# focegueda1998/CALM-ViT-DTE

Hardware: AMD Instinct MI355X
Metric: training images/sec (224^2, bs=256/GPU) (higher is better)
Workload: dtype f32; 1 GPU; CALM-ViT small224 cls, 224x224x3 synthetic, bs=256/GPU, fp32 matmuls, fwd+loss+bwd+clip+AdamW; batch resident in HBM when the timed region starts (the trainer's H2D copy of the batch is excluded); global_batch=256, parallelism=dp1, world=1, backend=none (single process), hipgraph=False

## Files before the change

calm-vit-dte_amd/_lib.py:

```python
import ctypes as C
import os

HERE = os.path.dirname(os.path.abspath(__file__))
LIB_PATH = os.environ.get("CALM_VIT_LIB") or os.path.join(HERE, "libcalmvit_hip.so")

ACT_NONE, ACT_GELU, ACT_GELU_BWD = 0, 1, 2
F32 = 0
ST_F32, ST_BF16, ST_FP8_E4M3, ST_FP8_E5M2 = 0, 1, 2, 3
E_INVAL, E_LAYOUT, E_UNSUPP = -1, -2, -3
ABI_VERSION = 7

_p = C.c_void_p
_i32 = C.c_int32
_i64 = C.c_int64
_f32 = C.c_float


class GemmArgs(C.Structure):
    _fields_ = [
        ("A", _p), ("B", _p), ("C", _p),
        ("M", _i32), ("N", _i32), ("K", _i32),
        ("batch0", _i32), ("batch1", _i32),
        ("a_rs", _i64), ("a_cs", _i64), ("a_b0", _i64), ("a_b1", _i64),
        ("b_rs", _i64), ("b_cs", _i64), ("b_b0", _i64), ("b_b1", _i64),
# ... 49 lines not shown
    "calm_gemm": (_i32, [C.POINTER(GemmArgs), _p]),
    "calm_gemm_workspace_bytes": (_i64, [C.POINTER(GemmArgs)]),
    "calm_gemm_set_option": (C.c_int, [_i32, _i32]),
    "calm_gemm_describe": (_i32, [C.POINTER(GemmArgs), C.POINTER(GemmPlan)]),
    "calm_reduce_scratch_floats": (_i64, [_i32, _i64, _i32]),
    "calm_layernorm_fwd": (_i32, [_p, _p, _p, _p, _p, _i64, _i32, _f32, _i32, _p]),
    "calm_layernorm_bwd": (_i32, [_p, _p, _p, _p, _p, _p, _p, _p, _i64, _i32, _i32, _p, _p]),
    "calm_cast_chunk_elems": (_i32, []),
    "calm_cast_bf16": (_i32, [_p, _p, _i32, _p]),
    "calm_cast_bf16_one": (_i32, [_p, _p, _i64, _p]),
    "calm_cast_f32_one": (_i32, [_p, _p, _i64, _p]),
    "calm_quantize_fp8": (_i32, [_p, _i32, _i64, _p, _i32, _p, _p]),
    "calm_transpose_u8": (_i32, [_p, _p, _i32, _i32, _p]),
    "calm_rope_fwd": (_i32, [_p, _p, _p, _p, _p, _i32, _i32, _i32, _i32, _i32, _i32, _i32, _i32, _p]),
    "calm_rope_bwd": (_i32, [_p, _p, _p, _p, _p, _p, _i32, _i32, _i32, _i32, _i32, _i32, _i32, _i32, _i32, _p, _p]),
    "calm_softmax_fwd": (_i32, [_p, _i64, _i32, _p]),
    "calm_softmax_bwd": (_i32, [_p, _p, _i64, _i32, _p]),
    "calm_softmax_bwd_heads": (_i32, [_p, _p, _p, _i32, _i32, _i32, _i32, _p]),
    "calm_sum_heads": (_i32, [_p, _p, _i32, _i32, _i64, _p]),
    "calm_attention_fwd_supported": (_i32, [_i32, _i32, _i32, _i32]),
    "calm_attention_fwd": (_i32, [_p] * 15 + [_i32] * 5 + [_p]),
    "calm_attention_bwd_preferred": (_i32, [_i32, _i32, _i32, _i32]),
    "calm_attention_bwd": (_i32, [_p] * 10 + [_i32] * 5 + [_p]),
    "calm_attention_fwd_lse": (_i32, [_p] * 15 + [_i32] * 5 + [_p]),
    "calm_attention_bwd_lse_scratch_bytes": (_i64, [_i32] * 5),
    "calm_attention_bwd_lse": (_i32, [_p] * 7 + [_i64] + [_p] * 4 + [_i32] * 5 + [_p]),
    "calm_attention16_supported": (_i32, [_i32, _i32, _i32]),
    "calm_attention16_fwd": (_i32, [_p] * 16 + [_i32] * 4 + [_p]),
    "calm_attention16_bwd": (_i32, [_p] * 13 + [_i32] * 4 + [_p]),
    "calm_latent_fwd": (_i32, [_p, _p, _p, _p, _p, _i64, _i32, _p, _p]),
    "calm_latent_bwd": (_i32, [_p, _p, _p, _p, _p, _p, _i64, _i32, _p]),
    "calm_sn_plan": (_i32, [C.POINTER(SnLayer), _i32, _p, C.POINTER(SnPlanInfo)]),
    "calm_sn_power_iter": (_i32, [_p, C.POINTER(SnPlanInfo), _i32, _f32, _p, _p]),
    "calm_sn_weight_bwd": (_i32, [_p, _p, _p, _p, _p, _p, _p, _p, _i32, _i32, _p, _p]),
    "calm_optim_chunk_elems": (_i32, []),
    "calm_optim_step": (_i32, [_p, _i32, _p, _i32, _p, C.POINTER(OptimHparams), _p, _p, _p, _p, _p]),
    "calm_collate_mix": (_i32, [_p, _p, _p, _i32, _i32, _i32, _i32, _f32, _p, _p, _p, _p]),
    "calm_collate_crop_mix": (_i32, [_p, _i32, _i32, _p, _p, _p, _i32, _i32, _i32, _i32, _i32, _f32, _p, _p, _p, _p]),
    "calm_image_to_rows": (_i32, [_p, _p, _i32, _i32, _p]),
    "calm_rows_to_image": (_i32, [_p, _p, _i32, _i32, _p]),
    "calm_grid_transpose": (_i32, [_p, _p, _i32, _i32, _p]),
    "calm_dwconv3x3_fwd": (_i32, [_p, _p, _p, _p, _p, _p, _i32, _i32, _i32, _i32, _p]),
    "calm_dwconv3x3_bwd": (_i32, [_p, _p, _p, _p, _p, _p, _p, _i32, _i32, _i32, _p]),
    "calm_cnn_residual_fwd": (_i32, [_p] * 11 + [_i32, _i32, _i32, _i32, _p]),
    "calm_cnn_residual_bwd": (_i32, [_p] * 18 + [_i32, _i32, _i32, _i32, _p, _p]),
    "calm_add": (_i32, [_p, _p, _p, _i64, _p]),
# ... 40 lines not shown
```

calm-vit-dte_amd/backend.py:

```python
import contextlib
import ctypes as C
import os

import numpy as np
import torch

from . import _lib
from ._lib import ACT_GELU, ACT_GELU_BWD, ACT_NONE

SN_EPS = 1e-12

GEMM_WORKSPACE = os.environ.get("CALM_GEMM_WORKSPACE", "1") != "0"
BF16_STORAGE = os.environ.get("CALM_BF16_STORAGE", "1") != "0"
PRECISIONS = {"fp32": 0, "bf16": 1, "bf16x3": 2, "fp8": 1}
FP8_DTYPES = (torch.float8_e4m3fn, torch.float8_e5m2)
_precision = "fp32"


def set_matmul_precision(name):
    global _precision
    if name not in PRECISIONS:
        raise ValueError(f"unknown matmul precision {name!r}; choose from {sorted(PRECISIONS)}")
    _precision = name

# ... 465 lines not shown
    def softmax_bwd_heads(self, p, dp, dm, B, H, Sq, cols):
        _lib.check(self.lib.calm_softmax_bwd_heads(_ptr(p), _ptr(dp), _ptr(dm), B, H, Sq, cols, _stream()),
                   "calm_softmax_bwd_heads")

    def sum_heads(self, dl, dm, B, H, per_head):
        _lib.check(self.lib.calm_sum_heads(_ptr(dl), _ptr(dm), B, H, per_head, _stream()), "calm_sum_heads")

    def attn_fwd_supported(self, Sq, Skv, H, hd):
        return bool(self.lib.calm_attention_fwd_supported(Sq, Skv, H, hd))

    def attn_fwd(self, q, k, v, w1, b1, s1, w2, b2, s2, out, R, hp, hg, Mk, P, B, Sq, Skv, H, hd):
        _lib.check(self.lib.calm_attention_fwd(_ptr(q), _ptr(k), _ptr(v), _ptr(w1), _ptr(b1), _ptr(s1), _ptr(w2),
                                               _ptr(b2), _ptr(s2), _ptr(out), _ptr(R), _ptr(hp), _ptr(hg),
                                               _ptr(Mk), _ptr(P, True), B, Sq, Skv, H, hd, _stream()), "calm_attention_fwd")

    def attn_bwd_preferred(self, Sq, Skv, H, hd):
        return bool(self.lib.calm_attention_bwd_preferred(Sq, Skv, H, hd))

    def attn_bwd(self, q, k, v, dout, P, dS, dq, dk, dv, dM, B, Sq, Skv, H, hd):
        _lib.check(self.lib.calm_attention_bwd(_ptr(q), _ptr(k), _ptr(v), _ptr(dout), _ptr(P), _ptr(dS), _ptr(dq),
                                               _ptr(dk), _ptr(dv), _ptr(dM), B, Sq, Skv, H, hd, _stream()),
                   "calm_attention_bwd")

    def attn_fwd_lse(self, q, k, v, w1, b1, s1, w2, b2, s2, out, R, hp, hg, Mk, lse, B, Sq, Skv, H, hd):
        _lib.check(self.lib.calm_attention_fwd_lse(_ptr(q), _ptr(k), _ptr(v), _ptr(w1), _ptr(b1), _ptr(s1), _ptr(w2),
                                                   _ptr(b2), _ptr(s2), _ptr(out), _ptr(R), _ptr(hp), _ptr(hg),
                                                   _ptr(Mk), _ptr(lse), B, Sq, Skv, H, hd, _stream()),
                   "calm_attention_fwd_lse")

    def attn_bwd_lse_scratch_bytes(self, B, Sq, Skv, H, hd):
        return int(self.lib.calm_attention_bwd_lse_scratch_bytes(B, Sq, Skv, H, hd))

    def attn_bwd_lse(self, q, k, v, dout, Mk, lse, scratch, dq, dk, dv, dM, B, Sq, Skv, H, hd):
        if scratch is None or not scratch.is_cuda or not scratch.is_contiguous():
            raise TypeError("attn_bwd_lse: contiguous CUDA scratch tensor expected")
        _lib.check(self.lib.calm_attention_bwd_lse(_ptr(q), _ptr(k), _ptr(v), _ptr(dout), _ptr(Mk), _ptr(lse),
                                                   scratch.data_ptr(), scratch.numel() * scratch.element_size(),
                                                   _ptr(dq), _ptr(dk), _ptr(dv), _ptr(dM), B, Sq, Skv, H, hd, _stream()),
                   "calm_attention_bwd_lse")

    def attn16_supported(self, S, H, hd):
        return bool(self.lib.calm_attention16_supported(S, H, hd))

    def attn16_fwd(self, q, k, v, w1, b1, s1, w2, b2, s2, out, R, hp, hg, Mk, MkT, lse, B, S, H, hd):
        h = lambda t: _ptr16(t)
        _lib.check(self.lib.calm_attention16_fwd(h(q), h(k), h(v), h(w1), _ptr(b1), _ptr(s1), h(w2), _ptr(b2), _ptr(s2),
# ... 147 lines not shown
```

calm-vit-dte_amd/csrc/attention_fused.hip:

```cpp
#include "common.h"

#ifndef ATT_TR_ROWFAST
#define ATT_TR_ROWFAST 1
#endif

namespace {

typedef float f32x4v __attribute__((ext_vector_type(4)));

struct AttnFwdP {
    const float* q; const float* k; const float* v;
    const float* w1; const float* b1; const float* s1;
    const float* w2; const float* b2; const float* s2;
    float* out;
    float* R; float* hp; float* hg; float* Mk; float* P;
    int B, Sq, Skv, H, hd;
    float scale;
    float* lse;
};

constexpr int NV_Q = 1;

template <int NV> struct Regs { f32x4v v[NV]; };

// ... 72 lines not shown
    static constexpr int NJ = NJ_, NW = NW_;
    static constexpr int SKV = 16 * NJ, TQ = 16 * NW;
    static constexpr int LDJ = ld_km(SKV), LDQ = ld_km(TQ);
    static constexpr int LDN1 = 20;
    static constexpr int LDJ2 = SKV + 4;
    static_assert(LDJ % 32 == 16 && LDQ % 32 == 16, "K-major strides: lane groups 16 banks apart");
    static constexpr int Q_OFF = 32 * LDJ, V_OFF = Q_OFF + 32 * LDQ;
    __device__ static float* buf_k(float* smem, int i) { return smem + i * 16 * LDJ; }
    __device__ static float* buf_q(float* smem, int i) { return smem + Q_OFF + i * 16 * LDQ; }
    static constexpr int W2_OFF = 2 * SKV * LDN1, PH2 = W2_OFF + 32 * LDJ2;
    __device__ static float* buf_w1(float* smem, int i) { return smem + i * SKV * LDN1; }
    __device__ static float* buf_w2(float* smem, int i) { return smem + W2_OFF + i * 16 * LDJ2; }
    struct Hd { int DT, hdp, LDV, stripe; };
    __host__ __device__ static constexpr Hd at(int hd) {
        const int DT = (hd + 15) / 16;
        const int hdp = 16 * DT, LDV = hdp + 4;
        return {DT, hdp, LDV, SKV * LDV};
    }
    static constexpr size_t fwd_bytes(int hd) {
        const int ph13 = V_OFF + at(hd).stripe;
        return sizeof(float) * (size_t)(ph13 > PH2 ? ph13 : PH2);
    }
    static constexpr size_t bwd_q_bytes(int hd) { return sizeof(float) * (size_t)(V_OFF + at(hd).stripe); }
    static constexpr size_t bwd_kv_bytes(int hd) { return sizeof(float) * (size_t)at(hd).stripe; }
};

template <int NJ, int NW>
__global__ __launch_bounds__(64 * NW) void attn_fwd_kernel(const AttnFwdP p) {
    constexpr int NTH = 64 * NW;
    constexpr int NV_K = (NJ + NW - 1) / NW;
    extern __shared__ __attribute__((aligned(16))) float smem[];
    typedef AttGeo<NJ, NW> G;
    constexpr int SKV = G::SKV, LDJ = G::LDJ, LDN1 = G::LDN1, LDJ2 = G::LDJ2;

    const int tid = threadIdx.x, lane = tid & 63, wave = tid >> 6;
    constexpr int TQ = G::TQ, LDQ = G::LDQ;
    const int r16 = lane & 15, g = lane >> 4;
    const int b = blockIdx.y;
    const int q0 = blockIdx.x * TQ;
    const int nq = min(TQ, p.Sq - q0);
    const bool active = 16 * wave < nq;
    const int iq = q0 + 16 * wave + r16;
    const int D = p.H * p.hd;

    const float* qb = p.q + ((long)b * p.Sq + q0) * D;
    const float* kb = p.k + (long)b * p.Skv * D;
    const float* vb = p.v + (long)b * p.Skv * D;
// ... 236 lines not shown
                    for (int r = 0; r < 4; ++r) {
                        accO = MFMA16(vcol[(16 * t + 4 * g + r) * LDV], accS[t][r], accO);
                        accO2 = MFMA16(vcol[(16 * t + 4 * g + r) * LDV + d2], accS[t][r], accO2);
                    }
                if (16 * d + 4 * g < hd) *reinterpret_cast<f32x4v*>(orow + 16 * d + 4 * g) = accO;
                if (d + 1 < DT && 16 * (d + 1) + 4 * g < hd)
                    *reinterpret_cast<f32x4v*>(orow + 16 * (d + 1) + 4 * g) = accO2;
            }
        }
        __syncthreads();
    }
}

struct AttnBwdP {
    const float* q; const float* k; const float* v; const float* dout;
    const float* P;
    float* dS;
    float* dq; float* dk; float* dv;
    float* dM;
    int B, Sq, Skv, H, hd;
    float scale;
    const float* Mk;
    const float* lse;
};

template <int NJ, int NW, bool LSE>
__global__ __launch_bounds__(64 * NW) void attn_bwd_q_kernel(const AttnBwdP p) {
    constexpr int NTH = 64 * NW;
    constexpr int NV_K = (NJ + NW - 1) / NW;
    extern __shared__ __attribute__((aligned(16))) float smem[];
    typedef AttGeo<NJ, NW> G;
    constexpr int SKV = G::SKV, LDJ = G::LDJ, TQ = G::TQ, LDQ = G::LDQ;
    const int tid = threadIdx.x, lane = tid & 63, wave = tid >> 6;
    const int r16 = lane & 15, g = lane >> 4;
    const int b = blockIdx.y;
    const int q0 = blockIdx.x * TQ;
    const int nq = min(TQ, p.Sq - q0);
    const bool active = 16 * wave < nq;
    const int iq = q0 + 16 * wave + r16;
    const int D = p.H * p.hd;
    const int hd = p.hd;
    const auto gh = G::at(hd);
    const int DT = gh.DT, hdp = gh.hdp, LDV = gh.LDV;
    auto bufK = [&](int i) { return G::buf_k(smem, i); };
    auto bufQ = [&](int i) { return G::buf_q(smem, i); };
    float* bufV = smem + G::V_OFF;
// ... 174 lines not shown
                const float* kcol = bufV + 16 * d + r16;
                const int d2 = (d + 1 < DT) ? 16 : 0;
#pragma unroll
                for (int t = 0; t < NJ; ++t)
#pragma unroll
                    for (int r = 0; r < 4; ++r) {
                        accO = MFMA16(kcol[(16 * t + 4 * g + r) * LDV], accD[t][r], accO);
                        accO2 = MFMA16(kcol[(16 * t + 4 * g + r) * LDV + d2], accD[t][r], accO2);
                    }
                if (16 * d + 4 * g < hd) *reinterpret_cast<f32x4v*>(qrow + 16 * d + 4 * g) = accO * p.scale;
                if (d + 1 < DT && 16 * (d + 1) + 4 * g < hd)
                    *reinterpret_cast<f32x4v*>(qrow + 16 * (d + 1) + 4 * g) = accO2 * p.scale;
            }
        }
        __syncthreads();
    }
    if (active) {
        float* mrow = p.dM + ((long)b * p.Sq + iq) * p.Skv;
#pragma unroll
        for (int t = 0; t < NJ; ++t) *reinterpret_cast<f32x4v*>(mrow + 16 * t + 4 * g) = accM[t];
    }
}

template <int NI, int NW>
__global__ __launch_bounds__(64 * NW) void attn_bwd_kv_kernel(const AttnBwdP p) {
    constexpr int NTH = 64 * NW;
    extern __shared__ __attribute__((aligned(16))) float smem[];
    typedef AttGeo<NI, NW> G;
    constexpr int SQ = G::SKV, TK = G::TQ;
    const int tid = threadIdx.x, lane = tid & 63, wave = tid >> 6;
    const int r16 = lane & 15, g = lane >> 4;
    const int b = blockIdx.y;
    const int k0 = blockIdx.x * TK;
    const int nk = min(TK, p.Skv - k0);
    const bool active = 16 * wave < nk;
    const int jk = k0 + 16 * wave + r16;
    const int D = p.H * p.hd;
    const int hd = p.hd;
    const auto gh = G::at(hd);
    const int DT = gh.DT, hdp = gh.hdp, LDV = gh.LDV;
    float* bufV = smem;
    const int v_per_row = hdp >> 2, v_total = SQ * v_per_row;
    const float* qb = p.q + (long)b * p.Sq * D;
    const float* dob = p.dout + (long)b * p.Sq * D;

    constexpr int SB = 4;
    auto stage = [&](const float* src) {
#pragma unroll 1
        for (int f0 = tid; f0 < v_total; f0 += SB * NTH) {
            f32x4v val[SB];
#pragma unroll
            for (int u = 0; u < SB; ++u) {
                const int f = f0 + u * NTH;
                const int row = f / v_per_row, cq = f - row * v_per_row;
                val[u] = (f32x4v){0.f, 0.f, 0.f, 0.f};
                if (f < v_total && 4 * cq < hd) val[u] = *reinterpret_cast<const f32x4v*>(src + (long)row * D + 4 * cq);
            }
#pragma unroll
            for (int u = 0; u < SB; ++u) {
                const int f = f0 + u * NTH;
                const int row = f / v_per_row, cq = f - row * v_per_row;
                if (f < v_total) *reinterpret_cast<f32x4v*>(bufV + row * LDV + 4 * cq) = val[u];
            }
        }
    };
    auto contract = [&](const f32x4v (&X)[NI], float* out_row, float scale) {
#pragma unroll 1
        for (int d = 0; d < DT; d += 2) {
            f32x4v accO = {0.f, 0.f, 0.f, 0.f}, accO2 = {0.f, 0.f, 0.f, 0.f};
            const float* col = bufV + 16 * d + r16;
            const int d2 = (d + 1 < DT) ? 16 : 0;
#pragma unroll
            for (int t = 0; t < NI; ++t)
#pragma unroll
                for (int r = 0; r < 4; ++r) {
                    accO = MFMA16(col[(16 * t + 4 * g + r) * LDV], X[t][r], accO);
                    accO2 = MFMA16(col[(16 * t + 4 * g + r) * LDV + d2], X[t][r], accO2);
                }
            if (16 * d + 4 * g < hd) *reinterpret_cast<f32x4v*>(out_row + 16 * d + 4 * g) = accO * scale;
            if (d + 1 < DT && 16 * (d + 1) + 4 * g < hd)
                *reinterpret_cast<f32x4v*>(out_row + 16 * (d + 1) + 4 * g) = accO2 * scale;
        }
    };

#pragma unroll 1
    for (int h = 0; h < p.H; ++h) {
        const long base = ((long)b * p.H + h) * p.Sq * p.Skv + (active ? jk : k0);
        f32x4v X[NI];
#pragma unroll
        for (int t = 0; t < NI; ++t)
#pragma unroll
            for (int r = 0; r < 4; ++r) X[t][r] = p.P[base + (long)(16 * t + 4 * g + r) * p.Skv];
        stage(dob + h * hd);
        __syncthreads();
        if (active) contract(X, p.dv + ((long)b * p.Skv + jk) * D + h * hd, 1.0f);
        __syncthreads();
#pragma unroll
        for (int t = 0; t < NI; ++t)
#pragma unroll
            for (int r = 0; r < 4; ++r) X[t][r] = p.dS[base + (long)(16 * t + 4 * g + r) * p.Skv];
        stage(qb + h * hd);
        __syncthreads();
        if (active) contract(X, p.dk + ((long)b * p.Skv + jk) * D + h * hd, p.scale);
        __syncthreads();
    }
}

template <class P>
int launch(void (*kernel)(const P), dim3 grid, int threads, size_t lds, hipStream_t s, const P& p) {
    hipError_t e = hipFuncSetAttribute(reinterpret_cast<const void*>(kernel), hipFuncAttributeMaxDynamicSharedMemorySize,
                                       (int)lds);
    if (e != hipSuccess) return (int)e;
    hipLaunchKernelGGL(kernel, grid, dim3(threads), lds, s, p);
    CALM_LAUNCH_CHECK();
    return 0;
}

template <class G, bool LSE>
int launch_bwd(const AttnBwdP& p, hipStream_t s) {
    static_assert(G::fwd_bytes(4) <= LDS_MAX, "fits at the smallest head dim; larger ones are checked per launch");
    constexpr int NJ = G::NJ, NW = G::NW;
    const int tiles = p.Sq / 16;
    dim3 grid((tiles + NW - 1) / NW, p.B);
    const int e = launch(&attn_bwd_q_kernel<NJ, NW, LSE>, grid, 64 * NW, G::bwd_q_bytes(p.hd), s, p);
    if (e) return e;
    return launch(&attn_bwd_kv_kernel<NJ, NW>, grid, 64 * NW, G::bwd_kv_bytes(p.hd), s, p);
}

template <class G>
int launch_fwd(const AttnFwdP& p, hipStream_t s) {
    static_assert(G::fwd_bytes(4) <= LDS_MAX, "fits at the smallest head dim; larger ones are checked per launch");
    constexpr int NJ = G::NJ, NW = G::NW;
    const int tiles = p.Sq / 16;
    const size_t lds = G::fwd_bytes(p.hd);
    if (lds > LDS_MAX) return CALM_E_UNSUPP;
    dim3 grid((tiles + NW - 1) / NW, p.B);
    return launch(&attn_fwd_kernel<NJ, NW>, grid, 64 * NW, lds, s, p);
}

#ifndef ATT_NW11
#define ATT_NW11 11
#endif
#ifndef ATT_NW14
#define ATT_NW14 7
#endif

template <class F>
int with_geo(int nj, F&& f) {
    switch (nj) {
// ... 43 lines not shown
                       float* hp, float* hg, float* Mk, float* P, int32_t B, int32_t Sq, int32_t Skv, int32_t H, int32_t hd,
                       void* stream) {
    return attention_fwd(q, k, v, w1, b1, s1, w2, b2, s2, out, R, hp, hg, Mk, P, nullptr, B, Sq, Skv, H, hd, stream);
}

int calm_attention_fwd_lse(const float* q, const float* k, const float* v, const float* w1, const float* b1,
                           const float* s1, const float* w2, const float* b2, const float* s2, float* out, float* R,
                           float* hp, float* hg, float* Mk, float* lse, int32_t B, int32_t Sq, int32_t Skv, int32_t H,
                           int32_t hd, void* stream) {
    if (!lse) return CALM_E_INVAL;
    return attention_fwd(q, k, v, w1, b1, s1, w2, b2, s2, out, R, hp, hg, Mk, nullptr, lse, B, Sq, Skv, H, hd, stream);
}

int calm_attention_bwd_preferred(int32_t Sq, int32_t Skv, int32_t H, int32_t hd) {
    return calm_attention_fwd_supported(Sq, Skv, H, hd) && (hd <= 64 || Skv / 16 == 11);
}

int calm_attention_bwd(const float* q, const float* k, const float* v, const float* dout, const float* P, float* dS,
                       float* dq, float* dk, float* dv, float* dM, int32_t B, int32_t Sq, int32_t Skv, int32_t H,
                       int32_t hd, void* stream) {
    if (!q || !k || !v || !dout || !P || !dS || !dq || !dk || !dv || !dM || B <= 0) return CALM_E_INVAL;
    if (!calm_attention_fwd_supported(Sq, Skv, H, hd)) return CALM_E_UNSUPP;
    if (B > 65535) return CALM_E_UNSUPP;
    AttnBwdP p{q, k, v, dout, P, dS, dq, dk, dv, dM, B, Sq, Skv, H, hd, 1.0f / sqrtf((float)hd), nullptr, nullptr};
    return attention_bwd_dispatch(p, false, as_stream(stream));
}

int64_t calm_attention_bwd_lse_scratch_bytes(int32_t B, int32_t Sq, int32_t Skv, int32_t H, int32_t hd) {
    if (B <= 0 || B > 65535 || !calm_attention_fwd_supported(Sq, Skv, H, hd)) return 0;
    return 2 * (int64_t)sizeof(float) * B * H * Sq * Skv;
}

int calm_attention_bwd_lse(const float* q, const float* k, const float* v, const float* dout, const float* Mk,
                           const float* lse, void* scratch, int64_t scratch_bytes, float* dq, float* dk, float* dv,
                           float* dM, int32_t B, int32_t Sq, int32_t Skv, int32_t H, int32_t hd, void* stream) {
    if (!q || !k || !v || !dout || !Mk || !lse || !scratch || !dq || !dk || !dv || !dM || B <= 0) return CALM_E_INVAL;
    const int64_t need = calm_attention_bwd_lse_scratch_bytes(B, Sq, Skv, H, hd);
    if (need == 0) return CALM_E_UNSUPP;
    if (scratch_bytes < need || (reinterpret_cast<uintptr_t>(scratch) & 15)) return CALM_E_INVAL;
    float* P = static_cast<float*>(scratch);
    float* dS = P + need / (2 * (int64_t)sizeof(float));
    AttnBwdP p{q, k, v, dout, P, dS, dq, dk, dv, dM, B, Sq, Skv, H, hd, 1.0f / sqrtf((float)hd), Mk, lse};
    return attention_bwd_dispatch(p, true, as_stream(stream));
}

}
```

calm-vit-dte_amd/ops.py:

```python
import math
import os
import threading

import torch
from torch.autograd import Function
from torch.autograd.function import once_differentiable

from .backend import (ACT_GELU, ACT_GELU_BWD, ACT_NONE, act_dtype, bf16_pipeline, fp8_linears, get_attention_storage,
                      get_backend)
from .spectral_norm import W16_ATTR, W16_GEN_ATTR

_amp_fwd = torch.amp.custom_fwd(device_type="cuda")
_amp_bwd = torch.amp.custom_bwd(device_type="cuda")

GROUP_PROJECTIONS = os.environ.get("CALM_GROUP_PROJECTIONS", "1") != "0"
FUSE_LN_SKIP = os.environ.get("CALM_FUSE_LN_SKIP", "1") != "0"

_noise_override = None


def set_noise_override(fn):
    global _noise_override
    _noise_override = fn

# ... 99 lines not shown
    return fp8_linears() and all(d % 16 == 0 for d in dims)


def _lin_fwd8(be, x2, w, sigma, out, **epi):
    M, K = x2.shape
    N = w.shape[0]
    xq, dqx = be.quantize_fp8(x2, E4M3)
    wq, dqw = be.quantize_fp8(_c(w), E4M3)
    be.gemm(xq, wq, out, M, N, K, (K, 1, 0, 0), (K, 1, 0, 0), (N, 0, 0), inv_scale=sigma, r=(N, 0, 0), split_k=1,
            a_dq=dqx, b_dq=dqw, **epi)


def _lin_dgrad8(be, dy2, w_eff, sigma, dx, **epi):
    M, N = dy2.shape
    K = w_eff.shape[1]
    dyq, dqd = be.quantize_fp8(dy2, E5M2)
    wq, dqw = be.quantize_fp8(_c(w_eff), E4M3)
    wtq = be.transpose_u8(wq)
    be.gemm(dyq, wtq, dx, M, K, N, (N, 1, 0, 0), (N, 1, 0, 0), (K, 0, 0), inv_scale=sigma, r=(K, 0, 0), split_k=1,
            a_dq=dqd, b_dq=dqw, **epi)


CAST_GRADS = os.environ.get("CALM_CAST_GRADS", "1") != "0"


def _gop(be, g2):
    if CAST_GRADS and bf16_pipeline() and g2.dtype == torch.float32 and g2.shape[-1] % 8 == 0 and g2.numel() >= (1 << 20):
        g16 = torch.empty(g2.shape, dtype=torch.bfloat16, device=g2.device)
        be.cast_bf16(g2, g16)
        return g16
    return g2


def _colsum(be, x2):
    out = _zeros((x2.shape[1],), x2 if x2.dtype == torch.float32 else x2.new_empty(0, dtype=torch.float32))
    be.colsum(x2, out, x2.shape[0], x2.shape[1])
    return out


class LayerNormFn(Function):

    @staticmethod
    @_amp_fwd
    def forward(ctx, x, w, eps, gemm_only=False):
        be = get_backend()
        x = _c(x)
# ... 308 lines not shown
        table = torch.empty(2 * S * (dr // 2), dtype=torch.float32, device=xr.device)
        out = torch.empty(B, S, H * (dc + dr), dtype=torch.bfloat16 if out16 else torch.float32, device=xr.device)
        be.rope_fwd(content, xr, inv_freq, table, out, B, S, H, dc, dr)
        ctx.dims = (B, S, H, dc, dr)
        ctx.content_dtype = content.dtype if content is not None else None
        ctx.save_for_backward(xr, table)
        return out

    @staticmethod
    @once_differentiable
    @_amp_bwd
    def backward(ctx, dout):
        be = get_backend()
        xr, table = ctx.saved_tensors
        B, S, H, dc, dr = ctx.dims
        dout = _c(dout)
        d_xr = torch.empty_like(xr)
        d_content = torch.empty(B, S, H * dc, dtype=ctx.content_dtype, device=xr.device) if dc > 0 else None
        d_if = _zeros((dr // 2,), table)
        be.rope_bwd(dout, xr, table, d_content, d_xr, d_if, B, S, H, dc, dr)
        return d_content, d_xr, d_if, None, None


def _attn_mask_bwd(be, defer, dM, q, k, dq, dk, R, hp, hg, w1, w2, u1, v1, s1, u2, v2, s2, w1o=None, w2o=None):
    w1o, w2o = w1 if w1o is None else w1o, w2 if w2o is None else w2o
    B, Sq, D = q.shape
    Skv = k.shape[1]
    dev, dt = q.device, q.dtype
    G2 = _zeros_big(w2.shape, w2)
    _lin_wgrad(be, dM, hg, G2)
    dW2, _ = _sn_wbwd(be, G2, w2, u2, v2, s2, defer=defer[1])
    db2 = _colsum(be, dM)
    dhp = torch.empty_like(hp)
    _lin_dgrad(be, dM, w2o, s2, dhp, act=ACT_GELU_BWD, aux=hp)
    R2 = R.view(B * Sq, Skv)
    G1 = _zeros_big(w1.shape, w1)
    _lin_wgrad(be, dhp, R2, G1)
    dW1, _ = _sn_wbwd(be, G1, w1, u1, v1, s1, defer=defer[0])
    db1 = _colsum(be, dhp)
    dR = torch.empty(B, Sq, Skv, dtype=dt, device=dev)
    _lin_dgrad(be, dhp, w1o, s1, dR.view(B * Sq, Skv))
    be.gemm(dR, k, dq, Sq, D, Skv, (Skv, 1, Sq * Skv, 0), (1, D, Skv * D, 0), (D, Sq * D, 0), batch=(B, 1),
            accumulate=True)
    be.gemm(dR, q, dk, Skv, D, Sq, (1, Skv, Sq * Skv, 0), (1, D, Sq * D, 0), (D, Skv * D, 0), batch=(B, 1),
            accumulate=True)
    return dW1, db1, dW2, db2


class LatentMaskAttentionFn(Function):

    @staticmethod
    @_amp_fwd
    def forward(ctx, q, k, v, w1, b1, w2, b2, u1, v1, s1, u2, v2, s2, H):
        be = get_backend()
        q, k, v = _c(q), _c(k), _c(v)
        B, Sq, D = q.shape
        Skv = k.shape[1]
        hd = D // H
        dev, dt = q.device, q.dtype
        R = torch.empty(B, Sq, Skv, dtype=dt, device=dev)
        hp = torch.empty(B * Sq, w1.shape[0], dtype=dt, device=dev)
        hg = torch.empty_like(hp)
        P = torch.empty(B, H, Sq, Skv, dtype=dt, device=dev)
        out = torch.empty(B, Sq, D, dtype=dt, device=dev)
        if be.attn_fwd_supported(Sq, Skv, H, hd):
            Mk = torch.empty(B * Sq, Skv, dtype=dt, device=dev)
# ... 12 lines not shown
                    batch=(B, H))
        ctx.H = H
        ctx.defer = (_deferred(w1), _deferred(w2))
        ctx.save_for_backward(q, k, v, R, hp, hg, P, w1, w2, u1, v1, s1, u2, v2, s2)
        return out

    @staticmethod
    @once_differentiable
    @_amp_bwd
    def backward(ctx, dout):
        be = get_backend()
        q, k, v, R, hp, hg, P, w1, w2, u1, v1, s1, u2, v2, s2 = ctx.saved_tensors
        H = ctx.H
        B, Sq, D = q.shape
        Skv = k.shape[1]
        hd = D // H
        scale = 1.0 / math.sqrt(hd)
        dout = _c(dout)
        dev, dt = q.device, q.dtype
        pb = (H * Sq * Skv, Sq * Skv)
        dP = torch.empty_like(P)
        dv, dq, dk = torch.empty_like(v), torch.empty_like(q), torch.empty_like(k)
        dM = torch.empty(B * Sq, Skv, dtype=dt, device=dev)
        if be.attn_bwd_preferred(Sq, Skv, H, hd):
            be.attn_bwd(q, k, v, dout, P, dP, dq, dk, dv, dM, B, Sq, Skv, H, hd)
        else:
            be.gemm(dout, v, dP, Sq, Skv, hd, (D, 1, Sq * D, hd), (D, 1, Skv * D, hd), (Skv,) + pb, batch=(B, H))
            be.gemm(P, dout, dv, Skv, hd, Sq, (1, Skv) + pb, (1, D, Sq * D, hd), (D, Skv * D, hd), batch=(B, H))
            be.softmax_bwd_heads(P, dP, dM, B, H, Sq, Skv)
            be.gemm(dP, k, dq, Sq, hd, Skv, (Skv, 1) + pb, (1, D, Skv * D, hd), (D, Sq * D, hd), batch=(B, H),
                    alpha=scale)
            be.gemm(dP, q, dk, Skv, hd, Sq, (1, Skv) + pb, (1, D, Sq * D, hd), (D, Skv * D, hd), batch=(B, H),
                    alpha=scale)
        dW1, db1, dW2, db2 = _attn_mask_bwd(be, ctx.defer, dM, q, k, dq, dk, R, hp, hg, w1, w2, u1, v1, s1, u2, v2, s2)
        return dq, dk, dv, dW1, db1, dW2, db2, None, None, None, None, None, None, None


class LatentMaskAttentionLseFn(Function):

    @staticmethod
    @_amp_fwd
    def forward(ctx, q, k, v, w1, b1, w2, b2, u1, v1, s1, u2, v2, s2, H):
        be = get_backend()
        q, k, v = _c(q), _c(k), _c(v)
        B, Sq, D = q.shape
        Skv = k.shape[1]
        hd = D // H
        dev, dt = q.device, q.dtype
        if not be.attn_fwd_supported(Sq, Skv, H, hd):
            raise RuntimeError(f"row-LSE attention: no fused kernel for Sq={Sq} Skv={Skv} H={H} hd={hd}")
        R = torch.empty(B, Sq, Skv, dtype=dt, device=dev)
        hp = torch.empty(B * Sq, w1.shape[0], dtype=dt, device=dev)
        hg = torch.empty_like(hp)
        Mk = torch.empty(B * Sq, Skv, dtype=dt, device=dev)
        lse = torch.empty(B, H, Sq, dtype=torch.float32, device=dev)
        out = torch.empty(B, Sq, D, dtype=dt, device=dev)
        be.attn_fwd_lse(q, k, v, w1, b1, s1, w2, b2, s2, out, R, hp, hg, Mk, lse, B, Sq, Skv, H, hd)
# ... 381 lines not shown
```

include/calm_vit.h:

```cpp
#ifndef CALM_VIT_H
#define CALM_VIT_H

#include <stddef.h>
#include <stdint.h>

#ifdef __cplusplus
extern "C" {
#endif

#define CALM_ABI_VERSION 7

#define CALM_E_INVAL   (-1)
#define CALM_E_LAYOUT  (-2)
#define CALM_E_UNSUPP  (-3)

enum { CALM_F32 = 0, CALM_BF16 = 1, CALM_BF16X3 = 2 };
enum { CALM_ST_F32 = 0, CALM_ST_BF16 = 1, CALM_ST_FP8_E4M3 = 2, CALM_ST_FP8_E5M2 = 3 };
enum { CALM_ACT_NONE = 0, CALM_ACT_GELU = 1, CALM_ACT_GELU_BWD = 2 };

int         calm_abi_version(void);
const char* calm_build_info(void);

typedef struct calm_gemm_args {
    const void* A; const void* B; void* C;
// ... 64 lines not shown
int calm_rope_bwd(const void* d_out, const void* xr, const float* table,
                  void* d_content, void* d_xr, float* d_inv_freq,
                  int32_t B, int32_t S, int32_t H, int32_t dc, int32_t dr,
                  int32_t dout_type, int32_t xr_type, int32_t dcontent_type, int32_t dxr_type,
                  float* partials , void* stream);

int calm_softmax_fwd(float* x, int64_t rows, int32_t cols, void* stream);
int calm_softmax_bwd(const float* p, float* dp, int64_t rows, int32_t cols, void* stream);
int calm_softmax_bwd_heads(const float* p, float* dp, float* dm, int32_t B, int32_t H, int32_t Sq, int32_t cols,
                           void* stream);
int calm_sum_heads(const float* dl, float* dm, int32_t B, int32_t H, int64_t per_head, void* stream);

int calm_attention_fwd_supported(int32_t Sq, int32_t Skv, int32_t H, int32_t hd);
int calm_attention_fwd(const float* q, const float* k, const float* v, const float* w1, const float* b1,
                       const float* s1, const float* w2, const float* b2, const float* s2, float* out, float* R,
                       float* hp, float* hg, float* Mk, float* P, int32_t B, int32_t Sq, int32_t Skv, int32_t H, int32_t hd,
                       void* stream);

int calm_attention_bwd_preferred(int32_t Sq, int32_t Skv, int32_t H, int32_t hd);
int calm_attention_bwd(const float* q, const float* k, const float* v, const float* dout, const float* P, float* dS,
                       float* dq, float* dk, float* dv, float* dM, int32_t B, int32_t Sq, int32_t Skv, int32_t H,
                       int32_t hd, void* stream);

int calm_attention_fwd_lse(const float* q, const float* k, const float* v, const float* w1, const float* b1,
                           const float* s1, const float* w2, const float* b2, const float* s2, float* out, float* R,
                           float* hp, float* hg, float* Mk, float* lse, int32_t B, int32_t Sq, int32_t Skv, int32_t H,
                           int32_t hd, void* stream);
int64_t calm_attention_bwd_lse_scratch_bytes(int32_t B, int32_t Sq, int32_t Skv, int32_t H, int32_t hd);
int calm_attention_bwd_lse(const float* q, const float* k, const float* v, const float* dout, const float* Mk,
                           const float* lse, void* scratch, int64_t scratch_bytes, float* dq, float* dk, float* dv,
                           float* dM, int32_t B, int32_t Sq, int32_t Skv, int32_t H, int32_t hd, void* stream);

int calm_attention16_supported(int32_t S, int32_t H, int32_t hd);
int calm_attention16_fwd(const void* q, const void* k, const void* v, const void* w1, const float* b1, const float* s1,
                         const void* w2, const float* b2, const float* s2, void* out, void* R, void* hp, void* hg,
                         void* Mk, void* MkT, float* lse, int32_t B, int32_t S, int32_t H, int32_t hd, void* stream);
int calm_attention16_bwd(const void* q, const void* k, const void* v, const void* out, const void* dout, const void* Mk,
                         const void* MkT, const float* lse, float* delta, void* dq, void* dk, void* dv, void* dM,
                         int32_t B, int32_t S, int32_t H, int32_t hd, void* stream);

int calm_latent_fwd(const float* mv, const float* noise, float* z, float* std_out, float* kl_sum,
                    int64_t rows, int32_t mvh, float* partials , void* stream);
int calm_latent_bwd(const float* dz, const float* d_kl_sum, const float* mv, const float* noise,
                    const float* std_in, float* dmv, int64_t rows, int32_t mvh, void* stream);

typedef struct calm_sn_layer {
// ... 111 lines not shown
```

Before: 1929 images/sec.

## Double-buffer attention dK/dV kernel via LDS DMA and add optional dR fold

Rewrites the attention backward K/V kernel to stage dout and q head slices into two LDS images with direct global-to-LDS loads. This overlaps the next head's load with the current contraction instead of syncing between stage and compute. It also splits the backward into separate q and kv entry points. An env-gated path folds the mask gradient dR into dS, so the separate dk GEMM in the mask backward is skipped. The added LDS footprint may lower occupancy, and the fold path is off by default.

```diff
diff --git a/calm-vit-dte_amd/_lib.py b/calm-vit-dte_amd/_lib.py
--- a/calm-vit-dte_amd/_lib.py
+++ b/calm-vit-dte_amd/_lib.py
@@ -95,6 +95,8 @@
     "calm_attention_fwd": (_i32, [_p] * 15 + [_i32] * 5 + [_p]),
     "calm_attention_bwd_preferred": (_i32, [_i32, _i32, _i32, _i32]),
     "calm_attention_bwd": (_i32, [_p] * 10 + [_i32] * 5 + [_p]),
+    "calm_attention_bwd_q": (_i32, [_p] * 8 + [_i32] * 5 + [_p]),
+    "calm_attention_bwd_kv": (_i32, [_p] * 7 + [_i32] * 5 + [_p]),
     "calm_attention_fwd_lse": (_i32, [_p] * 15 + [_i32] * 5 + [_p]),
     "calm_attention_bwd_lse_scratch_bytes": (_i64, [_i32] * 5),
     "calm_attention_bwd_lse": (_i32, [_p] * 7 + [_i64] + [_p] * 4 + [_i32] * 5 + [_p]),
diff --git a/calm-vit-dte_amd/backend.py b/calm-vit-dte_amd/backend.py
--- a/calm-vit-dte_amd/backend.py
+++ b/calm-vit-dte_amd/backend.py
@@ -511,6 +511,14 @@
                                                _ptr(dk), _ptr(dv), _ptr(dM), B, Sq, Skv, H, hd, _stream()),
                    "calm_attention_bwd")
 
+    def attn_bwd_q(self, q, k, v, dout, P, dS, dq, dM, B, Sq, Skv, H, hd):
+        _lib.check(self.lib.calm_attention_bwd_q(_ptr(q), _ptr(k), _ptr(v), _ptr(dout), _ptr(P), _ptr(dS), _ptr(dq),
+                                                 _ptr(dM), B, Sq, Skv, H, hd, _stream()), "calm_attention_bwd_q")
+
+    def attn_bwd_kv(self, q, dout, P, dS, dR, dk, dv, B, Sq, Skv, H, hd):
+        _lib.check(self.lib.calm_attention_bwd_kv(_ptr(q), _ptr(dout), _ptr(P), _ptr(dS), _ptr(dR, True), _ptr(dk),
+                                                  _ptr(dv), B, Sq, Skv, H, hd, _stream()), "calm_attention_bwd_kv")
+
     def attn_fwd_lse(self, q, k, v, w1, b1, s1, w2, b2, s2, out, R, hp, hg, Mk, lse, B, Sq, Skv, H, hd):
         _lib.check(self.lib.calm_attention_fwd_lse(_ptr(q), _ptr(k), _ptr(v), _ptr(w1), _ptr(b1), _ptr(s1), _ptr(w2),
                                                    _ptr(b2), _ptr(s2), _ptr(out), _ptr(R), _ptr(hp), _ptr(hg),
diff --git a/calm-vit-dte_amd/csrc/attention_fused.hip b/calm-vit-dte_amd/csrc/attention_fused.hip
--- a/calm-vit-dte_amd/csrc/attention_fused.hip
+++ b/calm-vit-dte_amd/csrc/attention_fused.hip
@@ -1,4 +1,5 @@
 #include "common.h"
+#include "lds_dma.h"
 
 #ifndef ATT_TR_ROWFAST
 #define ATT_TR_ROWFAST 1
@@ -118,7 +119,11 @@
         return sizeof(float) * (size_t)(ph13 > PH2 ? ph13 : PH2);
     }
     static constexpr size_t bwd_q_bytes(int hd) { return sizeof(float) * (size_t)(V_OFF + at(hd).stripe); }
-    static constexpr size_t bwd_kv_bytes(int hd) { return sizeof(float) * (size_t)at(hd).stripe; }
+    __host__ __device__ static constexpr int kv_image(int hd) { return (at(hd).stripe + 255) / 256 * 256; }
+    __host__ __device__ static constexpr int kv_images(int hd) {
+        return 2 * sizeof(float) * (size_t)((at(hd).stripe + 255) / 256 * 256) <= LDS_MAX ? 2 : 1;
+    }
+    static constexpr size_t bwd_kv_bytes(int hd) { return sizeof(float) * (size_t)(kv_images(hd) * kv_image(hd)); }
 };
 
 template <int NJ, int NW>
@@ -401,6 +406,7 @@
     float scale;
     const float* Mk;
     const float* lse;
+    const float* dR;
 };
 
 template <int NJ, int NW, bool LSE>
@@ -621,7 +627,7 @@
     }
 }
 
-template <int NI, int NW>
+template <int NI, int NW, bool FOLD>
 __global__ __launch_bounds__(64 * NW) void attn_bwd_kv_kernel(const AttnBwdP p) {
     constexpr int NTH = 64 * NW;
     extern __shared__ __attribute__((aligned(16))) float smem[];
@@ -638,10 +644,11 @@
     const int hd = p.hd;
     const auto gh = G::at(hd);
     const int DT = gh.DT, hdp = gh.hdp, LDV = gh.LDV;
-    float* bufV = smem;
     const int v_per_row = hdp >> 2, v_total = SQ * v_per_row;
     const float* qb = p.q + (long)b * p.Sq * D;
     const float* dob = p.dout + (long)b * p.Sq * D;
+    const float kscale = FOLD ? 1.0f : p.scale;
+    const int tile0 = (active ? jk : k0) + 4 * g * SQ;
 
     constexpr int SB = 4;
     auto stage = [&](const float* src) {
@@ -659,48 +666,119 @@
             for (int u = 0; u < SB; ++u) {
                 const int f = f0 + u * NTH;
                 const int row = f / v_per_row, cq = f - row * v_per_row;
-                if (f < v_total) *reinterpret_cast<f32x4v*>(bufV + row * LDV + 4 * cq) = val[u];
+                if (f < v_total) *reinterpret_cast<f32x4v*>(smem + row * LDV + 4 * cq) = val[u];
             }
         }
     };
-    auto contract = [&](const f32x4v (&X)[NI], float* out_row, float scale) {
+    const int ch_row = v_per_row + 1, n_chunks = SQ * ch_row, n_req = (n_chunks + 63) >> 6;
+    const int wave_u = __builtin_amdgcn_readfirstlane(wave);
+    const unsigned lds0 = (unsigned)__builtin_amdgcn_readfirstlane((int)(unsigned)reinterpret_cast<uintptr_t>(smem));
+    auto request = [&](const float* src, int image) {
+        const unsigned dst = lds0 + (unsigned)image * (unsigned)(sizeof(float) * G::kv_image(hd));
+#pragma unroll 1
+        for (int r = wave_u; r < n_req; r += NW) {
+            const int c = 64 * r + lane;
+            const int row = c / ch_row, cq = c - row * ch_row;
+            const float* a = reinterpret_cast<const float*>(calm_lds_dma::calm_zero_block);
+            if (c < n_chunks && 4 * cq < hd) a = src + (long)row * D + 4 * cq;
+            calm_lds_dma::glds16_addr(a, dst + 1024u * (unsigned)r);
+        }
+    };
+    auto landed = [&]() {
+        asm volatile("s_waitcnt vmcnt(0)" ::: "memory");
+        __builtin_amdgcn_s_barrier();
+        asm volatile("" ::: "memory");
+    };
+    auto contract = [&](const float* img, const f32x4v (&X)[NI], float* out_row, float scale) {
 #pragma unroll 1
         for (int d = 0; d < DT; d += 2) {
             f32x4v accO = {0.f, 0.f, 0.f, 0.f}, accO2 = {0.f, 0.f, 0.f, 0.f};
-            const float* col = bufV + 16 * d + r16;
             const int d2 = (d + 1 < DT) ? 16 : 0;
+            int ldv = LDV;
+            asm volatile("" : "+v"(ldv));
+            const float* col = img + 16 * d + r16 + 4 * g * ldv;
 #pragma unroll
             for (int t = 0; t < NI; ++t)
 #pragma unroll
                 for (int r = 0; r < 4; ++r) {
-                    accO = MFMA16(col[(16 * t + 4 * g + r) * LDV], X[t][r], accO);
-                    accO2 = MFMA16(col[(16 * t + 4 * g + r) * LDV + d2], X[t][r], accO2);
+                    accO = MFMA16(col[0], X[t][r], accO);
+                    accO2 = MFMA16(col[d2], X[t][r], accO2);
+                    col += (r < 3) ? ldv : 13 * ldv;
                 }
             if (16 * d + 4 * g < hd) *reinterpret_cast<f32x4v*>(out_row + 16 * d + 4 * g) = accO * scale;
             if (d + 1 < DT && 16 * (d + 1) + 4 * g < hd)
                 *reinterpret_cast<f32x4v*>(out_row + 16 * (d + 1) + 4 * g) = accO2 * scale;
         }
     };
-
+    auto load_tiles = [&](f32x4v (&X)[NI], const float* plane) {
+#pragma unroll
+        for (int t = 0; t < NI; ++t)
+#pragma unroll
+            for (int r = 0; r < 4; ++r) X[t][r] = plane[tile0 + (16 * t + r) * SQ];
+    };
+    auto load_ds = [&](f32x4v (&X)[NI], int h) {
+        load_tiles(X, p.dS + ((long)b * p.H + h) * p.Sq * p.Skv);
+        if constexpr (FOLD) {
+            constexpr int RG = (NI + 3) / 4, NG = (NI + RG - 1) / RG;
+            int t0 = tile0;
+            asm volatile("" : "+v"(t0));
+            const float* rp = p.dR + (long)b * p.Sq * p.Skv + t0;
+            f32x4v rt[2][RG];
+            auto load_group = [&](int gi) {
+#pragma unroll
+                for (int u = 0; u < RG; ++u)
+#pragma unroll
+                    for (int r = 0; r < 4; ++r)
+                        if (RG * gi + u < NI) rt[gi & 1][u][r] = rp[(16 * (RG * gi + u) + r) * SQ];
+            };
+            load_group(0);
+#pragma unroll
+            for (int gi = 0; gi < NG; ++gi) {
+                if (gi + 1 < NG) load_group(gi + 1);
+#pragma unroll
+                for (int u = 0; u < RG; ++u)
+                    if (RG * gi + u < NI) {
+                        f32x4v& x = X[RG * gi + u];
+#pragma unroll
+                        for (int r = 0; r < 4; ++r) x[r] = fmaf(x[r], p.scale, rt[gi & 1][u][r]);
+                        asm volatile("" : "+v"(x) :: "memory");
+                    }
+            }
+        }
+    };
+    float* dv_row = p.dv + ((long)b * p.Skv + jk) * D;
+    float* dk_row = p.dk + ((long)b * p.Skv + jk) * D;
+    f32x4v X[NI];
+
+    if (G::kv_images(hd) == 2) {
+        const float* img0 = smem;
+        const float* img1 = smem + G::kv_image(hd);
+        request(dob, 0);
+        load_tiles(X, p.P + (long)b * p.H * p.Sq * p.Skv);
+#pragma unroll 1
+        for (int h = 0; h < p.H; ++h) {
+            landed();
+            request(qb + h * hd, 1);
+            if (active) contract(img0, X, dv_row + h * hd, 1.0f);
+            load_ds(X, h);
+            landed();
+            if (h + 1 < p.H) request(dob + (h + 1) * hd, 0);
+            if (active) contract(img1, X, dk_row + h * hd, kscale);
+            if (h + 1 < p.H) load_tiles(X, p.P + ((long)b * p.H + h + 1) * p.Sq * p.Skv);
+        }
+        return;
+    }
 #pragma unroll 1
     for (int h = 0; h < p.H; ++h) {
-        const long base = ((long)b * p.H + h) * p.Sq * p.Skv + (active ? jk : k0);
-        f32x4v X[NI];
-#pragma unroll
-        for (int t = 0; t < NI; ++t)
-#pragma unroll
-            for (int r = 0; r < 4; ++r) X[t][r] = p.P[base + (long)(16 * t + 4 * g + r) * p.Skv];
+        load_tiles(X, p.P + ((long)b * p.H + h) * p.Sq * p.Skv);
         stage(dob + h * hd);
         __syncthreads();
-        if (active) contract(X, p.dv + ((long)b * p.Skv + jk) * D + h * hd, 1.0f);
+        if (active) contract(smem, X, dv_row + h * hd, 1.0f);
         __syncthreads();
-#pragma unroll
-        for (int t = 0; t < NI; ++t)
-#pragma unroll
-            for (int r = 0; r < 4; ++r) X[t][r] = p.dS[base + (long)(16 * t + 4 * g + r) * p.Skv];
+        load_ds(X, h);
         stage(qb + h * hd);
         __syncthreads();
-        if (active) contract(X, p.dk + ((long)b * p.Skv + jk) * D + h * hd, p.scale);
+        if (active) contract(smem, X, dk_row + h * hd, kscale);
         __syncthreads();
     }
 }
@@ -716,14 +794,26 @@
 }
 
 template <class G, bool LSE>
-int launch_bwd(const AttnBwdP& p, hipStream_t s) {
+int launch_bwd_q(const AttnBwdP& p, hipStream_t s) {
     static_assert(G::fwd_bytes(4) <= LDS_MAX, "fits at the smallest head dim; larger ones are checked per launch");
     constexpr int NJ = G::NJ, NW = G::NW;
-    const int tiles = p.Sq / 16;
-    dim3 grid((tiles + NW - 1) / NW, p.B);
-    const int e = launch(&attn_bwd_q_kernel<NJ, NW, LSE>, grid, 64 * NW, G::bwd_q_bytes(p.hd), s, p);
-    if (e) return e;
-    return launch(&attn_bwd_kv_kernel<NJ, NW>, grid, 64 * NW, G::bwd_kv_bytes(p.hd), s, p);
+    dim3 grid((p.Sq / 16 + NW - 1) / NW, p.B);
+    return launch(&attn_bwd_q_kernel<NJ, NW, LSE>, grid, 64 * NW, G::bwd_q_bytes(p.hd), s, p);
+}
+template <class G>
+int launch_bwd_kv(const AttnBwdP& p, hipStream_t s) {
+    static_assert(G::bwd_kv_bytes(4) <= LDS_MAX && G::kv_images(4) == 2, "two images at the smallest head dim");
+    constexpr int NJ = G::NJ, NW = G::NW;
+    const size_t lds = G::bwd_kv_bytes(p.hd);
+    if (lds > LDS_MAX) return CALM_E_UNSUPP;
+    dim3 grid((p.Sq / 16 + NW - 1) / NW, p.B);
+    return p.dR ? launch(&attn_bwd_kv_kernel<NJ, NW, true>, grid, 64 * NW, lds, s, p)
+                : launch(&attn_bwd_kv_kernel<NJ, NW, false>, grid, 64 * NW, lds, s, p);
+}
+template <class G, bool LSE>
+int launch_bwd(const AttnBwdP& p, hipStream_t s) {
+    const int e = launch_bwd_q<G, LSE>(p, s);
+    return e ? e : launch_bwd_kv<G>(p, s);
 }
 
 template <class G>
@@ -813,8 +903,30 @@
     if (!q || !k || !v || !dout || !P || !dS || !dq || !dk || !dv || !dM || B <= 0) return CALM_E_INVAL;
     if (!calm_attention_fwd_supported(Sq, Skv, H, hd)) return CALM_E_UNSUPP;
     if (B > 65535) return CALM_E_UNSUPP;
-    AttnBwdP p{q, k, v, dout, P, dS, dq, dk, dv, dM, B, Sq, Skv, H, hd, 1.0f / sqrtf((float)hd), nullptr, nullptr};
+    AttnBwdP p{q, k, v, dout, P, dS, dq, dk, dv, dM, B, Sq, Skv, H, hd, 1.0f / sqrtf((float)hd), nullptr, nullptr, nullptr};
     return attention_bwd_dispatch(p, false, as_stream(stream));
+}
+
+int calm_attention_bwd_q(const float* q, const float* k, const float* v, const float* dout, const float* P, float* dS,
+                         float* dq, float* dM, int32_t B, int32_t Sq, int32_t Skv, int32_t H, int32_t hd, void* stream) {
+    if (!q || !k || !v || !dout || !P || !dS || !dq || !dM || B <= 0) return CALM_E_INVAL;
+    if (!calm_attention_fwd_supported(Sq, Skv, H, hd)) return CALM_E_UNSUPP;
+    if (B > 65535) return CALM_E_UNSUPP;
+    AttnBwdP p{q, k, v, dout, P, dS, dq, nullptr, nullptr, dM, B, Sq, Skv, H, hd, 1.0f / sqrtf((float)hd), nullptr,
+               nullptr, nullptr};
+    hipStream_t s = as_stream(stream);
+    return with_geo(Skv / 16, [&](auto g) -> int { return launch_bwd_q<decltype(g), false>(p, s); });
+}
+
+int calm_attention_bwd_kv(const float* q, const float* dout, const float* P, const float* dS, const float* dR, float* dk,
+                          float* dv, int32_t B, int32_t Sq, int32_t Skv, int32_t H, int32_t hd, void* stream) {
+    if (!q || !dout || !P || !dS || !dk || !dv || B <= 0) return CALM_E_INVAL;
+    if (!calm_attention_fwd_supported(Sq, Skv, H, hd)) return CALM_E_UNSUPP;
+    if (B > 65535) return CALM_E_UNSUPP;
+    AttnBwdP p{q, nullptr, nullptr, dout, P, const_cast<float*>(dS), nullptr, dk, dv, nullptr, B, Sq, Skv, H, hd,
+               1.0f / sqrtf((float)hd), nullptr, nullptr, dR};
+    hipStream_t s = as_stream(stream);
+    return with_geo(Skv / 16, [&](auto g) -> int { return launch_bwd_kv<decltype(g)>(p, s); });
 }
 
 int64_t calm_attention_bwd_lse_scratch_bytes(int32_t B, int32_t Sq, int32_t Skv, int32_t H, int32_t hd) {
@@ -831,7 +943,7 @@
     if (scratch_bytes < need || (reinterpret_cast<uintptr_t>(scratch) & 15)) return CALM_E_INVAL;
     float* P = static_cast<float*>(scratch);
     float* dS = P + need / (2 * (int64_t)sizeof(float));
-    AttnBwdP p{q, k, v, dout, P, dS, dq, dk, dv, dM, B, Sq, Skv, H, hd, 1.0f / sqrtf((float)hd), Mk, lse};
+    AttnBwdP p{q, k, v, dout, P, dS, dq, dk, dv, dM, B, Sq, Skv, H, hd, 1.0f / sqrtf((float)hd), Mk, lse, nullptr};
     return attention_bwd_dispatch(p, true, as_stream(stream));
 }
 
diff --git a/calm-vit-dte_amd/ops.py b/calm-vit-dte_amd/ops.py
--- a/calm-vit-dte_amd/ops.py
+++ b/calm-vit-dte_amd/ops.py
@@ -145,6 +145,7 @@
 
 
 CAST_GRADS = os.environ.get("CALM_CAST_GRADS", "1") != "0"
+ATTN_BWD_FOLD = os.environ.get("CALM_ATTN_BWD_FOLD", "0") == "1"
 
 
 def _gop(be, g2):
@@ -499,7 +500,8 @@
         return d_content, d_xr, d_if, None, None
 
 
-def _attn_mask_bwd(be, defer, dM, q, k, dq, dk, R, hp, hg, w1, w2, u1, v1, s1, u2, v2, s2, w1o=None, w2o=None):
+def _attn_mask_bwd(be, defer, dM, q, k, dq, dk, R, hp, hg, w1, w2, u1, v1, s1, u2, v2, s2, w1o=None, w2o=None,
+                   dk_product=True):
     w1o, w2o = w1 if w1o is None else w1o, w2 if w2o is None else w2o
     B, Sq, D = q.shape
     Skv = k.shape[1]
@@ -519,6 +521,8 @@
     _lin_dgrad(be, dhp, w1o, s1, dR.view(B * Sq, Skv))
     be.gemm(dR, k, dq, Sq, D, Skv, (Skv, 1, Sq * Skv, 0), (1, D, Skv * D, 0), (D, Sq * D, 0), batch=(B, 1),
             accumulate=True)
+    if not dk_product:
+        return dW1, db1, dW2, db2, dR
     be.gemm(dR, q, dk, Skv, D, Sq, (1, Skv, Sq * Skv, 0), (1, D, Sq * D, 0), (D, Skv * D, 0), batch=(B, 1),
             accumulate=True)
     return dW1, db1, dW2, db2
@@ -577,6 +581,12 @@
         dP = torch.empty_like(P)
         dv, dq, dk = torch.empty_like(v), torch.empty_like(q), torch.empty_like(k)
         dM = torch.empty(B * Sq, Skv, dtype=dt, device=dev)
+        args = (ctx.defer, dM, q, k, dq, dk, R, hp, hg, w1, w2, u1, v1, s1, u2, v2, s2)
+        if be.attn_bwd_preferred(Sq, Skv, H, hd) and ATTN_BWD_FOLD and hasattr(be, "attn_bwd_kv"):
+            be.attn_bwd_q(q, k, v, dout, P, dP, dq, dM, B, Sq, Skv, H, hd)
+            dW1, db1, dW2, db2, dR = _attn_mask_bwd(be, *args, dk_product=False)
+            be.attn_bwd_kv(q, dout, P, dP, dR, dk, dv, B, Sq, Skv, H, hd)
+            return dq, dk, dv, dW1, db1, dW2, db2, None, None, None, None, None, None, None
         if be.attn_bwd_preferred(Sq, Skv, H, hd):
             be.attn_bwd(q, k, v, dout, P, dP, dq, dk, dv, dM, B, Sq, Skv, H, hd)
         else:
@@ -587,7 +597,7 @@
                     alpha=scale)
             be.gemm(dP, q, dk, Skv, hd, Sq, (1, Skv) + pb, (1, D, Sq * D, hd), (D, Skv * D, hd), batch=(B, H),
                     alpha=scale)
-        dW1, db1, dW2, db2 = _attn_mask_bwd(be, ctx.defer, dM, q, k, dq, dk, R, hp, hg, w1, w2, u1, v1, s1, u2, v2, s2)
+        dW1, db1, dW2, db2 = _attn_mask_bwd(be, *args)
         return dq, dk, dv, dW1, db1, dW2, db2, None, None, None, None, None, None, None
 
 
diff --git a/include/calm_vit.h b/include/calm_vit.h
--- a/include/calm_vit.h
+++ b/include/calm_vit.h
@@ -110,6 +110,11 @@
                        float* dq, float* dk, float* dv, float* dM, int32_t B, int32_t Sq, int32_t Skv, int32_t H,
                        int32_t hd, void* stream);
 
+int calm_attention_bwd_q(const float* q, const float* k, const float* v, const float* dout, const float* P, float* dS,
+                         float* dq, float* dM, int32_t B, int32_t Sq, int32_t Skv, int32_t H, int32_t hd, void* stream);
+int calm_attention_bwd_kv(const float* q, const float* dout, const float* P, const float* dS, const float* dR, float* dk,
+                          float* dv, int32_t B, int32_t Sq, int32_t Skv, int32_t H, int32_t hd, void* stream);
+
 int calm_attention_fwd_lse(const float* q, const float* k, const float* v, const float* w1, const float* b1,
                            const float* s1, const float* w2, const float* b2, const float* s2, float* out, float* R,
                            float* hp, float* hg, float* Mk, float* lse, int32_t B, int32_t Sq, int32_t Skv, int32_t H,
```

New measurement: 1938 images/sec, median of 6. No clear change (+0.5%).
